# kepengxu/PGTFormer

Hardware: NVIDIA H100
Metric: clips_per_s (higher is better)
Workload: dtype bf16

## Files before the change

include/pgt_b200.h:

```cpp
#ifndef PGT_B200_H_
#define PGT_B200_H_

#include <stdint.h>

#ifdef __cplusplus
extern "C" {
#endif

typedef enum pgt_status {
  PGT_OK = 0,
  PGT_ERR_INVALID = -1,
  PGT_ERR_CUDA = -2,
  PGT_ERR_UNSUPPORTED = -3,
  PGT_ERR_DRIVER = -4
} pgt_status;

enum { PGT_BF16 = 0, PGT_F32 = 1 };
enum { PGT_ACT_NONE = 0, PGT_ACT_GELU = 1, PGT_ACT_SILU = 2, PGT_ACT_LRELU02 = 3, PGT_ACT_RELU = 4,
       PGT_ACT_SIGMOID = 5 };
enum { PGT_EPI_PLAIN = 0,
       PGT_EPI_SFT = 1 };
enum { PGT_OUT_NHWC = 0, PGT_OUT_NCHW = 1 };
enum { PGT_EPI_FLAG_RELU_AFTER_RESIDUAL = 1 };

// ... 21 lines not shown
int64_t pgt_launch_count(void);
void pgt_reset_launch_count(void);
void pgt_tmap_cache_stats(int64_t* hits, int64_t* misses);

enum { PGT_PROF_GEMM = 0, PGT_PROF_WINDOW_ATTN = 1, PGT_PROF_MHA = 2, PGT_PROF_ARGMAX = 3, PGT_PROF_ARGMIN = 4,
       PGT_PROF_NORM = 5, PGT_PROF_MOVE = 6, PGT_PROF_LAYERNORM = 7, PGT_PROF_CLASSES = 8 };
int pgt_profile_begin(void);
int pgt_profile_end(double* work, double* ms, int64_t* launches);
int pgt_profile_end_csv(const char* path, double* work, double* ms, int64_t* launches);

int pgt_linear_bf16(const void* A, int lda, const void* W, int ldw, int M, int N, int K,
                    const pgt_epilogue* ep, void* stream);

int pgt_conv_bf16(const void* x, int F, int Hin, int Win, int Cin, int ldx, const void* Wp, int ldw,
                  int Cout, int ksize, int stride, int pad_lo, const pgt_epilogue* ep, void* stream);

int pgt_conv_out_gn(const void* x, int F, int H, int W, int Cin, int ldx, const float* gn_ab, const void* Wp, int ldw,
                    int Cout, const float* bias, float* out, void* stream);
int pgt_conv_out_gn_act(const void* x, int F, int H, int W, int Cin, int ldx, const float* gn_ab, const void* Wp, int ldw,
                        int Cout, const float* bias, float* out, int silu, void* stream);

int pgt_conv_up2x_bf16(const void* x, int F, int Hin, int Win, int Cin, int ldx, const void* Wp4, int ldw,
                       int Cout, const pgt_epilogue* ep, void* stream);

int pgt_conv_rgb_bf16(const float* x_nchw, int F, int H, int W, int ksize, int stride, int pad, const float* mean3,
                      const float* std3, const void* Wp, int ldw, int Cout, const float* bias, int act, void* out,
                      int ldo, float* gn_stats, void* stream);

int64_t pgt_groupnorm_ws_floats(int F, int HW, int C);
int pgt_conv_tiles_per_frame(int Hin, int Win, int Cout, int ksize, int stride, int pad_lo);
// ... 84 lines not shown
```

pgtformer_b200/_lib.py:

```python
import ctypes
import os
from ctypes import POINTER, Structure, c_char_p, c_float, c_int, c_int32, c_int64, c_void_p

HERE = os.path.dirname(os.path.abspath(__file__))
LIB_PATH = os.path.join(HERE, 'lib', 'libpgt_b200.so')

BF16, F32 = 0, 1
ACT_NONE, ACT_GELU, ACT_SILU, ACT_LRELU02, ACT_RELU, ACT_SIGMOID = 0, 1, 2, 3, 4, 5
EPI_PLAIN, EPI_SFT = 0, 1
OUT_NHWC, OUT_NCHW = 0, 1


class Epilogue(Structure):
    _fields_ = [('bias', c_void_p), ('act', c_int32), ('mode', c_int32), ('residual', c_void_p),
                ('ldr', c_int32), ('res_dtype', c_int32), ('aux', c_void_p), ('ldaux', c_int32),
                ('sft_w', c_float), ('out', c_void_p), ('ldo', c_int32), ('out_dtype', c_int32),
                ('out_layout', c_int32), ('flags', c_int32), ('gn_stats', c_void_p)]


SIGNATURES = {
    'pgt_strerror': (c_char_p, [c_int]),
    'pgt_last_cuda_error': (c_char_p, []),
    'pgt_version': (c_int, []),
    'pgt_launch_count': (c_int64, []),
    'pgt_reset_launch_count': (None, []),
    'pgt_tmap_cache_stats': (None, [c_void_p, c_void_p]),
    'pgt_profile_begin': (c_int, []),
    'pgt_profile_end': (c_int, [c_void_p, c_void_p, c_void_p]),
    'pgt_profile_end_csv': (c_int, [c_char_p, c_void_p, c_void_p, c_void_p]),
    'pgt_linear_bf16': (c_int, [c_void_p, c_int, c_void_p, c_int, c_int, c_int, c_int, POINTER(Epilogue), c_void_p]),
    'pgt_conv_bf16': (c_int, [c_void_p, c_int, c_int, c_int, c_int, c_int, c_void_p, c_int, c_int, c_int, c_int,
                              c_int, POINTER(Epilogue), c_void_p]),
    'pgt_conv_out_gn': (c_int, [c_void_p, c_int, c_int, c_int, c_int, c_int, c_void_p, c_void_p, c_int, c_int, c_void_p,
                                c_void_p, c_void_p]),
    'pgt_conv_out_gn_act': (c_int, [c_void_p, c_int, c_int, c_int, c_int, c_int, c_void_p, c_void_p, c_int, c_int,
                                    c_void_p, c_void_p, c_int, c_void_p]),
    'pgt_groupnorm_ab': (c_int, [c_void_p, c_int, c_int, c_int, c_int, c_void_p, c_void_p, c_float, c_void_p, c_int,
                                 c_void_p, c_void_p, c_void_p]),
    'pgt_conv_up2x_bf16': (c_int, [c_void_p, c_int, c_int, c_int, c_int, c_int, c_void_p, c_int, c_int,
                                   POINTER(Epilogue), c_void_p]),
    'pgt_conv_rgb_bf16': (c_int, [c_void_p, c_int, c_int, c_int, c_int, c_int, c_int, c_void_p, c_void_p, c_void_p, c_int,
                                  c_int, c_void_p, c_int, c_void_p, c_int, c_void_p, c_void_p]),
    'pgt_groupnorm_ws_floats': (c_int64, [c_int, c_int, c_int]),
    'pgt_conv_tiles_per_frame': (c_int, [c_int, c_int, c_int, c_int, c_int, c_int]),
    'pgt_conv_tiles_exact': (c_int, [c_int, c_int, c_int, c_int, c_int, c_int]),
    'pgt_groupnorm_apply_stats': (c_int, [c_void_p, c_int, c_int, c_int, c_int, c_void_p, c_void_p, c_float, c_int,
                                          c_void_p, c_int, c_void_p, c_int, c_void_p, c_void_p]),
    'pgt_groupnorm_silu': (c_int, [c_void_p, c_int, c_int, c_int, c_int, c_void_p, c_void_p, c_float, c_int,
# ... 83 lines not shown
```

pgtformer_b200/csrc/api.cu:

```cuda
#include <atomic>
#include <cstdio>
#include <cstring>
#include <vector>

#include "common.cuh"
#include "tmap.cuh"

namespace pgt {
static thread_local char g_last_error[512] = "";
static std::atomic<long long> g_launches{0};

void set_cuda_error(cudaError_t e, const char* where) {
  snprintf(g_last_error, sizeof(g_last_error), "%s: %s (%s)", where, cudaGetErrorName(e), cudaGetErrorString(e));
}
void count_launch(int n) { g_launches.fetch_add(n, std::memory_order_relaxed); }
int num_sms() {
  static std::atomic<int> per_dev[64];
  int dev = 0;
  if (cudaGetDevice(&dev) != cudaSuccess || dev < 0 || dev >= 64) return 132;
  int n = per_dev[dev].load(std::memory_order_relaxed);
  if (n == 0) {
    if (cudaDeviceGetAttribute(&n, cudaDevAttrMultiProcessorCount, dev) != cudaSuccess || n <= 0) n = 132;
    per_dev[dev].store(n, std::memory_order_relaxed);
  }
// ... 55 lines not shown
  pgt::g_prof.clear();
  return PGT_OK;
}

extern "C" const char* pgt_strerror(int status) {
  switch (status) {
    case PGT_OK: return "ok";
    case PGT_ERR_INVALID: return "invalid argument (shape / alignment / null pointer)";
    case PGT_ERR_CUDA: return "CUDA runtime error (see pgt_last_cuda_error)";
    case PGT_ERR_UNSUPPORTED: return "configuration not covered by the sm_90a kernels";
    case PGT_ERR_DRIVER: return "cuTensorMapEncodeTiled unavailable or failed";
    default: return "unknown status";
  }
}
extern "C" const char* pgt_last_cuda_error(void) { return pgt::g_last_error; }
extern "C" int pgt_version(void) { return 202; }
extern "C" void pgt_tmap_cache_stats(int64_t* hits, int64_t* misses) {
  long long h = 0, m = 0;
  pgt::tmap_cache_stats(&h, &m);
  if (hits) *hits = h;
  if (misses) *misses = m;
}
extern "C" int64_t pgt_launch_count(void) { return pgt::g_launches.load(); }
extern "C" void pgt_reset_launch_count(void) { pgt::g_launches.store(0); }
```

pgtformer_b200/csrc/gemm_tc.cu:

```cuda
#include <cudaTypedefs.h>
#include <cstdio>
#include <cstdlib>

#include "common.cuh"
#include "tmap.cuh"
#include "ptx.cuh"
#include "epi_common.cuh"

namespace pgt {

constexpr int BM = 128;
constexpr int BK = 64;
constexpr int EPI_WARPS = 8;
constexpr int GEMM_THREADS = EPI_WARPS * 32 + 128;
constexpr int PRODUCER_WARP = EPI_WARPS;
constexpr int DMA_WARP = EPI_WARPS + 1;
constexpr int CONSUMER_REGS = 232;
constexpr int PRODUCER_REGS = 40;
static_assert(2 * 128 * CONSUMER_REGS + 128 * PRODUCER_REGS <= 65536, "register file");
constexpr int XCH_LD = 68;
constexpr int XCH_BYTES = BM * XCH_LD * 4;
constexpr int XCH_WG_LD = 36;
constexpr int XCH_WG_BYTES = BM * XCH_WG_LD * 4;
constexpr int EPI_BAR = 1;
// ... 24 lines not shown
  int act, epi_mode;
  float* gn_stats;
  int gn_cpg;
  int ntaps, tap_kw, tap_oy, tap_ox;
  int gn_tpf;
  int gn_fstride;
  int relu_after_res;
  const void* residual;
  int ldr, res_dtype;
  const void* aux;
  int ldaux;
  float sft_w;
  void* out;
  int ldo, out_dtype, out_layout;
  double flops;
};

template <int BN>
struct GemmCfg {
  static constexpr int B_STAGE_BYTES = BN * BK * 2;
  static constexpr int STAGE_BYTES = A_STAGE_BYTES + B_STAGE_BYTES;
  static constexpr int SLOTS = staging_slots<BN>();
  static constexpr int STAGING_BYTES = SLOTS * PANEL_BYTES;
  static constexpr int BUDGET = 232448 - 1024  - STAGING_BYTES - XCH_BYTES - 256 ;
  static constexpr int STAGES = (BUDGET / STAGE_BYTES) > 6 ? 6 : (BUDGET / STAGE_BYTES);
  static constexpr int SMEM_BYTES = STAGES * STAGE_BYTES + STAGING_BYTES + XCH_BYTES + 256 + 1024;
  static_assert(SMEM_BYTES <= 232448, "gemm smem budget");
};

__device__ __forceinline__ void tile_mn(const GemmParams& p, int tile, int& m_blk, int& n_blk) {
// ... 632 lines not shown
constexpr int HALO_A_BYTES = (HALO_TH + 2) * HALO_PITCH;
constexpr int HALO_A_STRIDE = ((HALO_A_BYTES + 1023) / 1024) * 1024;

template <int BN>
struct HaloCfg {
  static constexpr int B_BYTES = BN * 128;
  static constexpr int A_STAGES = 2;
  static constexpr int B_STAGES = (BN == 64) ? 9 : 4;
  static constexpr int SLOTS = staging_slots<BN>();
  static constexpr int STAGING_BYTES = SLOTS * PANEL_BYTES;
  static constexpr int XCH = 2 * XCH_WG_BYTES;
  static constexpr int SMEM_BYTES = A_STAGES * HALO_A_STRIDE + B_STAGES * B_BYTES + STAGING_BYTES + XCH + 512 + 1024;
  static_assert(SMEM_BYTES <= 232448, "halo conv smem budget");
};

template <int S>
__device__ __forceinline__ void ring_skip(int& s, uint32_t& ph, int n) {
  const int t = s + n;
  ph ^= (uint32_t)(t / S) & 1u;
  s = t % S;
}

template <int BN>
__global__ void __launch_bounds__(GEMM_THREADS, 1)
conv_halo_kernel(const __grid_constant__ CUtensorMap tmA, const __grid_constant__ CUtensorMap tmB,
                 const __grid_constant__ CUtensorMap tmO, const __grid_constant__ CUtensorMap tmR,
                 const __grid_constant__ CUtensorMap tmX, const GemmParams p) {
  using Cfg = HaloCfg<BN>;
  constexpr int AS = Cfg::A_STAGES, BS = Cfg::B_STAGES;
  constexpr int RELEASERS = 4;
  extern __shared__ uint8_t smem_raw[];
  uint8_t* smem = reinterpret_cast<uint8_t*>((reinterpret_cast<uintptr_t>(smem_raw) + 1023) & ~uintptr_t(1023));
  uint8_t* smem_a = smem;
  uint8_t* smem_b = smem + AS * HALO_A_STRIDE;
  uint8_t* staging = smem_b + BS * Cfg::B_BYTES;
  float* xch = reinterpret_cast<float*>(staging + Cfg::STAGING_BYTES);
  uint64_t* bars = reinterpret_cast<uint64_t*>(staging + Cfg::STAGING_BYTES + Cfg::XCH);
  uint64_t* a_full = bars;
  uint64_t* a_empty = bars + AS;
  uint64_t* b_full = bars + 2 * AS;
  uint64_t* b_empty = bars + 2 * AS + BS;
  uint64_t* res_bar = bars + 2 * AS + 2 * BS;
  uint64_t* slot_ready = res_bar + Cfg::SLOTS;

  const int warp = threadIdx.x >> 5;
  const int lane = threadIdx.x & 31;
  const int num_tiles = p.m_tiles * p.n_tiles;
  const int cin_pad = p.cin_blocks * BK;

  if (warp == PRODUCER_WARP && lane == 0) {
    tma_prefetch_desc(&tmA);
    tma_prefetch_desc(&tmB);
    if (p.fast_epi) tma_prefetch_desc(&tmO);
    if (p.has_res_map) tma_prefetch_desc(&tmR);
    if (p.fast_epi && p.epi_mode == PGT_EPI_SFT) tma_prefetch_desc(&tmX);
    for (int i = 0; i < AS; ++i) { mbar_init(&a_full[i], 1); mbar_init(&a_empty[i], RELEASERS); }
    for (int i = 0; i < BS; ++i) { mbar_init(&b_full[i], 1); mbar_init(&b_empty[i], RELEASERS); }
    for (int i = 0; i < Cfg::SLOTS; ++i) {
      mbar_init(&res_bar[i], 1);
      mbar_init(&slot_ready[i], RELEASERS * 32);
    }
    fence_barrier_init();
  }
  __syncthreads();

  if (warp >= EPI_WARPS) {
    setmaxnreg_dec<PRODUCER_REGS>();
    if (warp == PRODUCER_WARP) {
      int as = 0, bs = 0;
      uint32_t aph = 0, bph = 0;
      for (int tile = blockIdx.x; tile < num_tiles; tile += gridDim.x) {
        const int n_blk = tile % p.n_tiles;
        const int m_blk = tile / p.n_tiles;
        int n0, y0, x0;
        decode_conv_tile(p, m_blk, n0, y0, x0);
        {
          const int pt = tile + PREFETCH_TILES * (int)gridDim.x;
          if (BN == 64 && pt < num_tiles && elect_one()) {
            int pn0, py0, px0;
            decode_conv_tile(p, pt / p.n_tiles, pn0, py0, px0);
            for (int cb = 0; cb < p.cin_blocks; ++cb) tma_prefetch_4d(&tmA, cb * BK, px0 - 1, py0 - 1, pn0);
            if (p.has_res_map) {
              const int c0 = (pt % p.n_tiles) * BN;
              const int rw = p.out_dtype == PGT_BF16 ? 64 : 32;
              for (int c = 0; c < BN && c0 + c < p.N; c += rw) {
                tma_prefetch_4d(&tmR, c0 + c, px0, py0, pn0);
                if (p.epi_mode == PGT_EPI_SFT) tma_prefetch_4d(&tmX, c0 + c, px0, py0, pn0);
              }
            }
          }
          __syncwarp();
        }
        for (int cb = 0; cb < p.cin_blocks; ++cb) {
          mbar_wait(&a_empty[as], aph ^ 1);
          if (elect_one()) {
            mbar_arrive_expect_tx(&a_full[as], HALO_A_BYTES);
            tma_load_4d(smem_a + as * HALO_A_STRIDE, &tmA, &a_full[as], cb * BK, x0 - 1, y0 - 1, n0);
          }
          __syncwarp();
          if (++as == AS) { as = 0; aph ^= 1; }
          if (p.b_resident && tile != (int)blockIdx.x) continue;
          for (int t = 0; t < p.ntaps; ++t) {
            mbar_wait(&b_empty[bs], bph ^ 1);
            if (elect_one()) {
              mbar_arrive_expect_tx(&b_full[bs], Cfg::B_BYTES);
              tma_load_2d(smem_b + bs * Cfg::B_BYTES, &tmB, &b_full[bs], t * cin_pad + cb * BK, n_blk * BN);
            }
            __syncwarp();
            if (++bs == BS) { bs = 0; bph ^= 1; }
          }
        }
      }
      for (int i = 0; i < AS; ++i) {
        mbar_wait(&a_empty[as], aph ^ 1);
        if (++as == AS) { as = 0; aph ^= 1; }
      }
    } else if (warp == DMA_WARP) {
      const EpiCtx ctx{staging, xch, res_bar, slot_ready};
      epilogue_dma_loop<BN>(p, ctx, tmO, tmR, tmX, lane, num_tiles);
    }
  } else {
    setmaxnreg_inc<CONSUMER_REGS>();
    const int wg = warp >> 2;
    const EpiCtx ctx{staging, xch + wg * (XCH_WG_BYTES / 4), res_bar, slot_ready};
    const uint32_t a_base = smem_u32(smem_a);
    const uint32_t b_base = smem_u32(smem_b);
    constexpr uint64_t ROW_BLOCK = 8 * HALO_PITCH / 16;
    const ItemStream<BN> is(p, num_tiles);
    const int b_per_tile = p.b_resident ? 0 : p.ntaps * p.cin_blocks;
    int as = 0, bs = 0;
    uint32_t aph = 0, bph = 0;
    int k = 0;
    bool first = true;
    for (int tile = blockIdx.x, j = 0; tile < num_tiles; tile += gridDim.x, ++j) {
      const bool has_next = tile + (int)gridDim.x < num_tiles;
      const int items = p.fast_epi ? is.panels_in_tile(tile) : 0;
      if ((j & 1) != wg) {
// ... 150 lines not shown
  }
  PGT_LAUNCH_OK();
  return PGT_OK;
}

template <int BN>
static int launch_halo(const CUtensorMap& tmA, const void* W, int ldw, GemmParams& p, cudaStream_t stream) {
  using Cfg = HaloCfg<BN>;
  CUtensorMap tmB, tmO, tmR, tmX;
  int rc = encode_weight_map(&tmB, W, ldw, p.K, p.N, BN);
  if (rc != PGT_OK) return rc;
  rc = setup_epilogue_maps(p, tmA, tmO, tmR, tmX);
  if (rc != PGT_OK) return rc;
  p.n_tiles = ceil_div(p.N, BN);
  p.b_resident = (p.ntaps * p.cin_blocks <= Cfg::B_STAGES && p.n_tiles == 1) ? 1 : 0;
  static PerDeviceOnce once;
  PGT_CUDA_OK(once.run([] { return cudaFuncSetAttribute(conv_halo_kernel<BN>, cudaFuncAttributeMaxDynamicSharedMemorySize, Cfg::SMEM_BYTES); }));
  const int tiles = p.m_tiles * p.n_tiles;
  const int grid = tiles < num_sms() ? tiles : num_sms();
  {
    char desc[96];
    if (prof_enabled())
      snprintf(desc, sizeof(desc), "halo3 F%d H%d W%d K%d N%d BN%d e%d r%d", p.F, p.H, p.W, p.K, p.N, BN, p.fast_epi,
               p.b_resident);
    ProfScope ps(PGT_PROF_GEMM, p.flops, stream, desc);
    conv_halo_kernel<BN><<<grid, GEMM_THREADS, Cfg::SMEM_BYTES, stream>>>(tmA, tmB, tmO, tmR, tmX, p);
  }
  PGT_LAUNCH_OK();
  return PGT_OK;
}

static bool wide_tiles(const GemmParams& p) {
  if (p.N <= 128 || p.num_kb < 8 || p.epi_mode == PGT_EPI_SFT) return false;
  if (ceil_div(p.N, 256) * 256 > ceil_div(p.N, 128) * 128) return false;
  return p.m_tiles * ceil_div(p.N, 256) >= num_sms();
}

static int dispatch_gemm(const CUtensorMap& tmA, const void* W, int ldw, GemmParams& p, cudaStream_t stream) {
  if (p.N <= 64) return launch_gemm<64>(tmA, W, ldw, p, stream);
  if (wide_tiles(p)) return launch_gemm<256>(tmA, W, ldw, p, stream);
  return launch_gemm<128>(tmA, W, ldw, p, stream);
// ... 37 lines not shown
  p.M = M; p.N = N; p.K = K;
  p.num_kb = ceil_div(K, BK);
  p.m_tiles = ceil_div(M, BM);
  p.flops = 2.0 * M * (double)N * K;
  int rc = fill_epilogue(p, ep);
  if (rc != PGT_OK) return rc;
  CUtensorMap tmA;
  uint64_t dims[2] = {(uint64_t)K, (uint64_t)M};
  uint64_t str[1] = {(uint64_t)lda * 2};
  uint32_t box[2] = {BK, BM};
  rc = encode_map(&tmA, A, 2, dims, str, box);
  if (rc != PGT_OK) return rc;
  return dispatch_gemm(tmA, W, ldw, p, static_cast<cudaStream_t>(stream));
}

static int conv_impl(const void* x, int F, int Hin, int Win, int Cin, int ldx, const void* Wp, int ldw, int Cout,
                     int ksize, int stride, int pad_y, int pad_x, int up_phase, const pgt_epilogue* ep, void* stream) {
  const int pad_lo = pad_y;
  PGT_CHECK_ARG(x && Wp && F > 0 && Hin > 0 && Win > 0 && Cin > 0 && Cout > 0);
  PGT_CHECK_ARG((ksize >= 1 && ksize <= 3) && (stride == 1 || stride == 2) && pad_y >= 0 && pad_y <= 1 && pad_x >= 0 && pad_x <= 1);
  PGT_CHECK_ARG(stride == 1 || (ksize != 2 && pad_x == pad_y));
  PGT_CHECK_ARG((ldx % 8) == 0 && (ldw % 8) == 0 && aligned16(x) && aligned16(Wp) && ldx >= Cin);
  const int cin_pad = ceil_div(Cin, BK) * BK;
  PGT_CHECK_ARG(ldw >= ksize * ksize * cin_pad);
  GemmParams p{};
  p.N = Cout;
  p.ksize = ksize;
  p.pad_lo = pad_lo;
  p.pad_x = pad_x; p.pad_y = pad_y;
  p.cin_blocks = cin_pad / BK;
  p.K = ksize * ksize * cin_pad;
  p.num_kb = ksize * ksize * p.cin_blocks;
// ... 8 lines not shown
    p.mode = MODE_CONV_S2;
    p.H = Hin / 2; p.W = Win / 2;
    p.cin_ld = ldx;
  }
  rc = fill_epilogue(p, ep);
  if (rc != PGT_OK) return rc;
  if (up_phase >= 0) {
    if (stride != 1 || p.out_layout != PGT_OUT_NHWC || p.epi_mode != PGT_EPI_PLAIN || p.residual != nullptr)
      return PGT_ERR_UNSUPPORTED;
    const int py = up_phase >> 1, px = up_phase & 1;
    const int esz = p.out_dtype == PGT_BF16 ? 2 : 4;
    const long long Wo = 2LL * Win;
    p.out = static_cast<char*>(p.out) + ((long long)py * Wo + px) * p.ldo * esz;
    p.o_sx = 2LL * p.ldo; p.o_sy = 2LL * Wo * p.ldo; p.o_sf = 4LL * Hin * Win * p.ldo;
  }
  static const bool no_halo = getenv("PGT_NO_HALO") != nullptr;
  const bool halo = !no_halo && stride == 1 && Cout <= 128 && Hin >= HALO_TH && Win >= HALO_TW &&
                    ((up_phase < 0 && ksize == 3 && pad_y == 1 && pad_x == 1) || (up_phase >= 0 && ksize == 2));
  p.ntaps = ksize * ksize; p.tap_kw = ksize;
  p.tap_oy = up_phase >= 0 ? (up_phase >> 1) : 0;
  p.tap_ox = up_phase >= 0 ? (up_phase & 1) : 0;
  int tw = 1, th = 1, tn;
  if (halo) {
    tw = HALO_TW; th = HALO_TH;
  } else {
    while (tw * 2 <= p.W && tw * 2 <= BM) tw *= 2;
    while (th * 2 <= p.H && tw * th * 2 <= BM) th *= 2;
  }
  tn = BM / (tw * th);
  p.tw = tw; p.th = th; p.tn = tn;
  p.tiles_x = ceil_div(p.W, tw);
  p.tiles_y = ceil_div(p.H, th);
  p.m_tiles = p.tiles_x * p.tiles_y * ceil_div(F, tn);
// ... 51 lines not shown
}

extern "C" int pgt_conv_tiles_exact(int Hin, int Win, int Cout, int ksize, int stride, int pad_lo) {
  int tw, th;
  if (!conv_tile_shape(Hin, Win, Cout, ksize, stride, pad_lo, tw, th)) return 0;
  const int H = Hin / stride, W = Win / stride;
  return (W % tw == 0 && H % th == 0) ? (W / tw) * (H / th) : 0;
}

extern "C" int pgt_conv_bf16(const void* x, int F, int Hin, int Win, int Cin, int ldx, const void* Wp, int ldw,
                             int Cout, int ksize, int stride, int pad_lo, const pgt_epilogue* ep, void* stream) {
  PGT_CHECK_ARG(ksize == 1 || ksize == 3);
  return conv_impl(x, F, Hin, Win, Cin, ldx, Wp, ldw, Cout, ksize, stride, pad_lo, pad_lo, -1, ep, stream);
}

extern "C" int pgt_conv_up2x_bf16(const void* x, int F, int Hin, int Win, int Cin, int ldx, const void* Wp4, int ldw,
                                  int Cout, const pgt_epilogue* ep, void* stream) {
  PGT_CHECK_ARG(Wp4 != nullptr && ldw > 0);
  const int cin_pad = ceil_div(Cin, BK) * BK;
  PGT_CHECK_ARG(ldw >= 4 * cin_pad);
  for (int ph = 0; ph < 4; ++ph) {
    const int py = ph >> 1, px = ph & 1;
    const void* w = static_cast<const char*>(Wp4) + (size_t)ph * Cout * ldw * 2;
    int rc = conv_impl(x, F, Hin, Win, Cin, ldx, w, ldw, Cout, 2, 1, 1 - py, 1 - px, ph, ep, stream);
    if (rc != PGT_OK) return rc;
  }
  return PGT_OK;
}
```

pgtformer_b200/csrc_torch/pgt_torch_ops.cpp:

```cpp
#include <ATen/ATen.h>
#include <ATen/cuda/CUDAContext.h>
#include <c10/cuda/CUDAGuard.h>
#include <torch/library.h>

#include "../../include/pgt_b200.h"

namespace {

void check(int rc, const char* what) {
  if (rc == PGT_OK) return;
  std::string msg = std::string("libpgt_b200 (") + what + "): " + pgt_strerror(rc);
  if (rc == PGT_ERR_CUDA) msg += std::string(": ") + pgt_last_cuda_error();
  TORCH_CHECK(false, msg);
}

void* stream_of(const at::Tensor& t) { return at::cuda::getCurrentCUDAStream(t.device().index()).stream(); }

int ld(const at::Tensor& t) {
  TORCH_CHECK(t.stride(-1) == 1, "expected a channels-last tensor");
  return t.dim() > 1 ? (int)t.stride(-2) : (int)t.size(-1);
}

void window_attention(const at::Tensor& qkv, int64_t clips, int64_t H, int64_t W, int64_t C, int64_t heads, int64_t shift,
                      const at::Tensor& tab16, at::Tensor out) {
// ... 141 lines not shown
                     const c10::optional<at::Tensor>& bias, bool silu, at::Tensor out) {
  TORCH_CHECK(x.is_cuda() && x.dim() == 4 && x.scalar_type() == at::kBFloat16 && x.stride(3) == 1 &&
              x.stride(1) == x.size(2) * x.stride(2) && (x.size(0) == 1 || x.stride(0) == x.size(1) * x.stride(1)) &&
              ab.scalar_type() == at::kFloat && wp.scalar_type() == at::kBFloat16 && wp.stride(1) == 1 &&
              out.scalar_type() == at::kFloat && out.is_contiguous() && out.dim() == 4 && out.size(0) == x.size(0) &&
              out.size(1) == cout && out.size(2) == x.size(1) && out.size(3) == x.size(2),
              "conv_out_gn_act: bf16 x [F, H, W, 64], fp32 ab [F, 2, 64], bf16 packed wp, fp32 out [F, cout, H, W]");
  TORCH_CHECK(ab.device() == x.device() && wp.device() == x.device() && out.device() == x.device() &&
              (!bias.has_value() || (bias->device() == x.device() && bias->scalar_type() == at::kFloat)),
              "conv_out_gn_act: every tensor on x's device, fp32 bias");
  c10::cuda::CUDAGuard guard(x.device());
  check(pgt_conv_out_gn_act(x.data_ptr(), (int)x.size(0), (int)x.size(1), (int)x.size(2), (int)x.size(3), (int)x.stride(2),
                            ab.data_ptr<float>(), wp.data_ptr(), (int)wp.stride(0), (int)cout,
                            bias.has_value() ? bias->data_ptr<float>() : nullptr, out.data_ptr<float>(), silu ? 1 : 0,
                            stream_of(x)), "conv_out_gn_act");
}

void vq_stats(const at::Tensor& z, const at::Tensor& codebook, const at::Tensor& idx, int64_t HW, double beta,
              at::Tensor scalars, const c10::optional<at::Tensor>& zq_nchw, const c10::optional<at::Tensor>& zq_bf16,
              const c10::optional<at::Tensor>& min_enc, const c10::optional<at::Tensor>& scores,
              const c10::optional<at::Tensor>& usage) {
  TORCH_CHECK(z.is_cuda() && z.dim() == 2 && z.scalar_type() == at::kFloat && z.is_contiguous() &&
              codebook.scalar_type() == at::kFloat && codebook.is_contiguous() && codebook.dim() == 2 &&
              codebook.size(1) == z.size(1) && idx.scalar_type() == at::kLong && idx.is_contiguous() &&
              idx.numel() == z.size(0) && scalars.scalar_type() == at::kFloat && scalars.is_contiguous() &&
              scalars.numel() >= 3, "vq_stats: fp32 z [T, E], codebook [K, E], int64 idx [T], fp32 scalars [3]");
  const int64_t T = z.size(0), E = z.size(1), K = codebook.size(0);
  TORCH_CHECK(codebook.device() == z.device() && idx.device() == z.device() && scalars.device() == z.device(),
              "vq_stats: codebook, idx and scalars must be on z's device");
  auto opt = [&z](const c10::optional<at::Tensor>& t, at::ScalarType dt, int64_t n) -> void* {
// ... 20 lines not shown

TORCH_LIBRARY(pgt, m) {
  m.def("window_attention(Tensor qkv, int clips, int H, int W, int C, int heads, int shift, Tensor tab16, Tensor(a!) out) -> ()");
  m.def("mha_fwd(Tensor q, Tensor k, Tensor v, int clips, int L, int heads, int d, Tensor(a!) out) -> ()");
  m.def("argmax_gather(Tensor logits, Tensor codebook, Tensor(a!) idx, Tensor(b!) quant) -> ()");
  m.def("codebook_pack(Tensor codebook, int K) -> (Tensor, Tensor)");
  m.def("l2_argmin(Tensor z, Tensor codebook, Tensor cb16, Tensor norm, int K, Tensor(a!) idx, Tensor(b!)? quant) -> ()");
  m.def("l2_argmin_split(Tensor z, Tensor codebook, Tensor cb16, Tensor norm, int K, int splits, Tensor(a!) idx, "
        "Tensor(b!)? quant) -> ()");
  m.def("linear(Tensor a, Tensor w, Tensor? bias, int act, Tensor? residual, Tensor(a!) out) -> ()");
  m.def("soft_codes(Tensor z, Tensor codebook, Tensor norm, int K, float temp, Tensor(a!) out) -> ()");
  m.def("sample_codes(Tensor p, Tensor seed, Tensor(a!) idx) -> ()");
  m.def("rq_residual(Tensor? r_in, Tensor(a!)? r_out, Tensor idx, Tensor codebook, Tensor(b!)? agg, bool first) -> ()");
  m.def("rq_embed(Tensor idx, int d0, int d1, Tensor codebooks, Tensor(a!) out, int ldi, int ldd) -> ()");
  m.def("conv_out_gn_act(Tensor x, Tensor ab, Tensor wp, int cout, Tensor? bias, bool silu, Tensor(a!) out) -> ()");
  m.def("vq_stats(Tensor z, Tensor codebook, Tensor idx, int HW, float beta, Tensor(a!) scalars, Tensor(b!)? zq_nchw, "
        "Tensor(c!)? zq_bf16, Tensor(d!)? min_enc, Tensor(e!)? scores, Tensor(f!)? usage) -> ()");
}

TORCH_LIBRARY_IMPL(pgt, CUDA, m) {
  m.impl("window_attention", window_attention);
  m.impl("mha_fwd", mha_fwd);
  m.impl("argmax_gather", argmax_gather);
  m.impl("codebook_pack", codebook_pack);
  m.impl("l2_argmin", l2_argmin);
  m.impl("l2_argmin_split", l2_argmin_split);
  m.impl("linear", linear);
  m.impl("soft_codes", soft_codes);
  m.impl("sample_codes", sample_codes);
  m.impl("rq_residual", rq_residual);
  m.impl("rq_embed", rq_embed);
  m.impl("conv_out_gn_act", conv_out_gn_act);
  m.impl("vq_stats", vq_stats);
}
```

pgtformer_b200/engine.py:

```python
import torch
import torch.nn.functional as F

from . import ops
from .spec import Arch
from .swin3d import pack_blocks

BF = torch.bfloat16


def _on_device(fn):
    import functools

    @functools.wraps(fn)
    def wrapper(self, *a, **k):
        with torch.cuda.device(self.dev):
            return fn(self, *a, **k)
    return wrapper


def _pack_conv(w):
    co, ci, kh, kw = w.shape
    cp = (ci + 63) // 64 * 64
    wp = torch.zeros(co, kh * kw, cp, dtype=torch.float32, device=w.device)
    wp[:, :, :ci] = w.permute(0, 2, 3, 1).reshape(co, kh * kw, ci)
# ... 132 lines not shown
    def _gn_stats(self, out, chunks_per_frame):
        if chunks_per_frame <= 0 or not ops.gn_stats_supported(out.shape[-1]) or not out.is_contiguous():
            return None
        stats = self._new(out.shape[0] * chunks_per_frame * 64, dtype=torch.float32)
        out._pgt_gn = (stats, chunks_per_frame)
        return stats

    def _gn(self, x, p, silu=True):
        gn = getattr(x, '_pgt_gn', None)
        if gn is not None:
            return ops.groupnorm_apply_stats(x, self.w[p + '.weight'], self.w[p + '.bias'], self._new(*x.shape), gn[0], gn[1],
                                             silu=silu)
        return ops.groupnorm_silu(x, self.w[p + '.weight'], self.w[p + '.bias'], self._new(*x.shape), silu=silu)

    def _conv3(self, x, p, cout, out=None, gn_out=False, gn=None, gn_silu=True, **kw):
        Fr, H, W, _ = x.shape
        stride = kw.get('stride', 1)
        if gn is not None:
            x = self._gn(x, gn, silu=gn_silu)
        if out is None:
            out = self._new(Fr, H // stride, W // stride, cout)
        stats = None
        if gn_out:
            stats = self._gn_stats(out, 4 * self._stats_tiles(H, W, cout, kw.get('ksize', 3), stride, kw.get('pad_lo', 1)))
        return ops.conv(x, self.w[p + '.weight'], cout, out, bias=self.w.get(p + '.bias'), gn_stats=stats, **kw)

    def _lin(self, x, p, n, out=None, out_dtype=BF, gn_out=False, **kw):
        if out is None:
            out = self._new(*x.shape[:-1], n, dtype=out_dtype)
        stats = None
        if gn_out and out.dim() == 4 and out.dtype == BF and (out.shape[1] * out.shape[2]) % 128 == 0:
            stats = self._gn_stats(out, out.shape[1] * out.shape[2] // 32)
        return ops.linear(x, self.w[p + '.weight'], out, bias=self.w.get(p + '.bias'), N=n, gn_stats=stats, **kw)

    def td_resblock(self, x, p, cout, gn_next=False, out=None, shortcut='nin_shortcut'):
        h = self._conv3(x, p + '.conv1', cout, gn=p + '.norm1', gn_out=True)
        sc = self._lin(x, p + '.' + shortcut, cout) if (p + '.' + shortcut + '.weight') in self.w else x
        return self._conv3(h, p + '.conv2', cout, gn=p + '.norm2', residual=sc, gn_out=gn_next, out=out)

# ... 516 lines not shown
```

pgtformer_b200/ops.py:

```python
import ctypes

import torch

from . import _lib as L
from ._lib import (ACT_GELU, ACT_LRELU02, ACT_NONE, ACT_RELU, ACT_SIGMOID, ACT_SILU, BF16, EPI_PLAIN,
                   EPI_SFT, F32, OUT_NCHW, OUT_NHWC, Epilogue)


def _p(t):
    return ctypes.c_void_p(t.data_ptr()) if t is not None else None


def _stream(t=None):
    if t is not None:
        return ctypes.c_void_p(torch.cuda.current_stream(t.device).cuda_stream)
    return ctypes.c_void_p(torch.cuda.current_stream().cuda_stream)


def _dt(t):
    if t.dtype == torch.bfloat16:
        return BF16
    if t.dtype == torch.float32:
        return F32
    raise TypeError('unsupported dtype %s' % t.dtype)
# ... 58 lines not shown
    return out


def conv(x, wp, cout, out, ksize=3, stride=1, pad_lo=1, bias=None, act=ACT_NONE, residual=None, sft_scale=None,
         sft_w=0.0, nchw=False, relu_after_res=False, gn_stats=None):
    lib = L.load()
    F, H, W, Cin = x.shape
    assert x.dtype == torch.bfloat16 and x.stride(3) == 1 and x.stride(1) == W * x.stride(2) and \
        (F == 1 or x.stride(0) == H * x.stride(1))
    ep = make_epilogue(out, bias, act, residual, sft_scale, sft_w, nchw, relu_after_res, gn_stats)
    L.check(lib.pgt_conv_bf16(_p(x), F, H, W, Cin, x.stride(2), _p(wp), wp.stride(0), cout, ksize, stride, pad_lo,
                              ctypes.byref(ep), _stream()))
    return out


def conv_rgb(x_nchw, wp, bias, out, ksize, stride, pad, act=ACT_NONE, mean3=None, std3=None, gn_stats=None):
    lib = L.load()
    F, C, H, W = x_nchw.shape
    assert C == 3 and x_nchw.dtype == torch.float32 and x_nchw.is_contiguous() and wp.dtype == torch.bfloat16
    m = (ctypes.c_float * 3)(*[float(v) for v in mean3]) if mean3 is not None else None
    s = (ctypes.c_float * 3)(*[float(v) for v in std3]) if std3 is not None else None
    L.check(lib.pgt_conv_rgb_bf16(_p(x_nchw), F, H, W, ksize, stride, pad, m, s, _p(wp), wp.stride(0), wp.shape[0],
                                  _p(bias), act, _p(out), _rows(out)[2], _p(gn_stats), _stream()))
    return out


def conv_up2x(x, wp4, cout, out, bias=None, act=ACT_NONE, gn_stats=None):
    lib = L.load()
    F, H, W, Cin = x.shape
    assert x.dtype == torch.bfloat16 and wp4.dtype == torch.bfloat16 and wp4.is_contiguous() and wp4.dim() == 3
# ... 438 lines not shown
```

Measured before the change: 90.60.

## Fuse GroupNorm+SiLU on the input into the halo conv via a slab-builder warpgroup

Adds a GN variant of the halo conv kernel. An extra 128-thread builder warpgroup loads raw bf16 activations, applies the per-frame GroupNorm affine (a,b) and SiLU (as a tanh form), and writes the swizzled halo slab into shared memory instead of using a TMA load. The engine computes only the GN coefficients and skips materialising the normalised tensor for Cout<=64 3x3 convs. This removes a full read/write pass over the activations, but the extra threads raise register pressure and the SiLU math moves onto the conv's A-operand critical path.

```diff
diff --git a/include/pgt_b200.h b/include/pgt_b200.h
--- a/include/pgt_b200.h
+++ b/include/pgt_b200.h
@@ -59,6 +59,11 @@
 
 int pgt_conv_bf16(const void* x, int F, int Hin, int Win, int Cin, int ldx, const void* Wp, int ldw,
                   int Cout, int ksize, int stride, int pad_lo, const pgt_epilogue* ep, void* stream);
+
+int pgt_conv_gn_supported(int Hin, int Win, int Cin, int Cout, int ksize, int stride, int pad_lo);
+int pgt_conv_gn_bf16(const void* x, int F, int Hin, int Win, int Cin, int ldx, const void* Wp, int ldw, int Cout,
+                     int ksize, int stride, int pad_lo, const float* in_ab, int in_silu, const pgt_epilogue* ep,
+                     void* stream);
 
 int pgt_conv_out_gn(const void* x, int F, int H, int W, int Cin, int ldx, const float* gn_ab, const void* Wp, int ldw,
                     int Cout, const float* bias, float* out, void* stream);
diff --git a/pgtformer_b200/_lib.py b/pgtformer_b200/_lib.py
--- a/pgtformer_b200/_lib.py
+++ b/pgtformer_b200/_lib.py
@@ -31,7 +31,10 @@
     'pgt_linear_bf16': (c_int, [c_void_p, c_int, c_void_p, c_int, c_int, c_int, c_int, POINTER(Epilogue), c_void_p]),
     'pgt_conv_bf16': (c_int, [c_void_p, c_int, c_int, c_int, c_int, c_int, c_void_p, c_int, c_int, c_int, c_int,
                               c_int, POINTER(Epilogue), c_void_p]),
-    'pgt_conv_out_gn': (c_int, [c_void_p, c_int, c_int, c_int, c_int, c_int, c_void_p, c_void_p, c_int, c_int, c_void_p,
+    'pgt_conv_gn_supported': (c_int, [c_int, c_int, c_int, c_int, c_int, c_int, c_int]),
+    'pgt_conv_gn_bf16': (c_int, [c_void_p, c_int, c_int, c_int, c_int, c_int, c_void_p, c_int, c_int, c_int, c_int,
+                                 c_int, c_void_p, c_int, POINTER(Epilogue), c_void_p]),
+    'pgt_conv_out_gn':(c_int, [c_void_p, c_int, c_int, c_int, c_int, c_int, c_void_p, c_void_p, c_int, c_int, c_void_p,
                                 c_void_p, c_void_p]),
     'pgt_conv_out_gn_act': (c_int, [c_void_p, c_int, c_int, c_int, c_int, c_int, c_void_p, c_void_p, c_int, c_int,
                                     c_void_p, c_void_p, c_int, c_void_p]),
diff --git a/pgtformer_b200/csrc/api.cu b/pgtformer_b200/csrc/api.cu
--- a/pgtformer_b200/csrc/api.cu
+++ b/pgtformer_b200/csrc/api.cu
@@ -93,7 +93,7 @@
   }
 }
 extern "C" const char* pgt_last_cuda_error(void) { return pgt::g_last_error; }
-extern "C" int pgt_version(void) { return 202; }
+extern "C" int pgt_version(void) { return 203; }
 extern "C" void pgt_tmap_cache_stats(int64_t* hits, int64_t* misses) {
   long long h = 0, m = 0;
   pgt::tmap_cache_stats(&h, &m);
diff --git a/pgtformer_b200/csrc/gemm_tc.cu b/pgtformer_b200/csrc/gemm_tc.cu
--- a/pgtformer_b200/csrc/gemm_tc.cu
+++ b/pgtformer_b200/csrc/gemm_tc.cu
@@ -62,6 +62,9 @@
   void* out;
   int ldo, out_dtype, out_layout;
   double flops;
+  const __nv_bfloat16* gn_x;
+  const float* gn_ab;
+  int gn_ldx, gn_cin, gn_silu;
 };
 
 template <int BN>
@@ -724,6 +727,142 @@
   static_assert(SMEM_BYTES <= 232448, "halo conv smem budget");
 };
 
+constexpr int HALO_GN_THREADS = GEMM_THREADS + 128;
+constexpr int HALO_GN_BUILDER_WARP = EPI_WARPS + 4;
+constexpr int HALO_GN_CONSUMER_REGS = 168;
+static_assert(2 * 128 * HALO_GN_CONSUMER_REGS + 128 * PRODUCER_REGS + 128 * (65536 / HALO_GN_THREADS) <= 65536,
+              "register file");
+constexpr int HALO_SLAB_PIX = (HALO_TH + 2) * (HALO_TW + 2);
+constexpr int GN_SLOTS = 12;
+
+__device__ __forceinline__ int opaque(int v) {
+  asm volatile("" : "+r"(v));
+  return v;
+}
+
+template <int L, int PART>
+__device__ __forceinline__ void gn_slab_load(const GemmParams& p, int n0, int y0, int x0, int cb, int bt, uint4 (&r)[L],
+                                             uint32_t& mask) {
+  const int ch = cb * BK + (bt & 7) * 8;
+  const int prow = opaque(bt >> 3);
+  mask = 0;
+#pragma unroll
+  for (int j = 0; j < L; ++j) {
+    const int pix = prow + 16 * (PART * L + j);
+    const int sy = pix / (HALO_TW + 2), sx = pix - sy * (HALO_TW + 2);
+    const int y = y0 - 1 + sy, x = x0 - 1 + sx;
+    r[j] = make_uint4(0, 0, 0, 0);
+    if (ch < p.gn_cin && pix < HALO_SLAB_PIX && (unsigned)y < (unsigned)p.H && (unsigned)x < (unsigned)p.W) {
+      r[j] = __ldg(reinterpret_cast<const uint4*>(p.gn_x + ((size_t)(n0 * p.H + y) * p.W + x) * p.gn_ldx + ch));
+      mask |= 1u << j;
+    }
+  }
+}
+
+template <int L>
+__device__ __forceinline__ void gn_slab_convert(const GemmParams& p, uint4 (&r)[L], uint32_t mask, const float (&a)[8],
+                                                const float (&b)[8]) {
+#pragma unroll
+  for (int j = 0; j < L; ++j) {
+    uint4 o = make_uint4(0, 0, 0, 0);
+    if (mask & (1u << j)) {
+      const uint32_t u[4] = {r[j].x, r[j].y, r[j].z, r[j].w};
+      uint32_t q[4];
+#pragma unroll
+      for (int e = 0; e < 4; ++e) {
+        const float2 xv = unpack_bf16x2(u[e]);
+        float h0 = fmaf(xv.x, a[2 * e], b[2 * e]), h1 = fmaf(xv.y, a[2 * e + 1], b[2 * e + 1]);
+        if (p.gn_silu) {
+          float t0, t1;
+          asm("tanh.approx.f32 %0, %1;" : "=f"(t0) : "f"(h0));
+          asm("tanh.approx.f32 %0, %1;" : "=f"(t1) : "f"(h1));
+          h0 = fmaf(h0, t0, h0);
+          h1 = fmaf(h1, t1, h1);
+        }
+        q[e] = pack_bf16x2(h0, h1);
+      }
+      o = make_uint4(q[0], q[1], q[2], q[3]);
+    }
+    r[j] = o;
+  }
+}
+
+template <int L>
+__device__ __forceinline__ void gn_slab_store(uint32_t slab, int bt, const uint4 (&r)[L]) {
+  const int chunk = bt & 7;
+  const int prow = opaque(bt >> 3);
+#pragma unroll
+  for (int j = 0; j < L; ++j) {
+    const int pix = prow + 16 * j;
+    if (pix < HALO_SLAB_PIX) sts128(slab + pix * 128 + ((chunk ^ (pix & 7)) << 4), r[j]);
+  }
+}
+
+template <int BN>
+__device__ __forceinline__ void halo_l2_prefetch(const GemmParams& p, const CUtensorMap& tmA, const CUtensorMap& tmR,
+                                                 const CUtensorMap& tmX, int tile, int num_tiles) {
+  const int pt = tile + PREFETCH_TILES * (int)gridDim.x;
+  if (BN == 64 && pt < num_tiles && elect_one()) {
+    int pn0, py0, px0;
+    decode_conv_tile(p, pt / p.n_tiles, pn0, py0, px0);
+    for (int cb = 0; cb < p.cin_blocks; ++cb) tma_prefetch_4d(&tmA, cb * BK, px0 - 1, py0 - 1, pn0);
+    if (p.has_res_map) {
+      const int c0 = (pt % p.n_tiles) * BN;
+      const int rw = p.out_dtype == PGT_BF16 ? 64 : 32;
+      for (int c = 0; c < BN && c0 + c < p.N; c += rw) {
+        tma_prefetch_4d(&tmR, c0 + c, px0, py0, pn0);
+        if (p.epi_mode == PGT_EPI_SFT) tma_prefetch_4d(&tmX, c0 + c, px0, py0, pn0);
+      }
+    }
+  }
+  __syncwarp();
+}
+
+template <int BN>
+__device__ __forceinline__ void gn_slab_builder(const GemmParams& p, const CUtensorMap& tmA, const CUtensorMap& tmR,
+                                                const CUtensorMap& tmX, uint8_t* smem_a, uint64_t* a_full,
+                                                uint64_t* a_empty, int num_tiles) {
+  const int bt = threadIdx.x - HALO_GN_BUILDER_WARP * 32;
+  const int ch = (bt & 7) * 8;
+  int as = 0;
+  uint32_t aph = 0;
+  for (int tile = blockIdx.x; tile < num_tiles; tile += gridDim.x) {
+    if (bt < 32) halo_l2_prefetch<BN>(p, tmA, tmR, tmX, tile, num_tiles);
+    int n0, y0, x0;
+    decode_conv_tile(p, tile / p.n_tiles, n0, y0, x0);
+    for (int cb = 0; cb < p.cin_blocks; ++cb) {
+      uint4 r[GN_SLOTS];
+      uint32_t mask;
+      gn_slab_load<GN_SLOTS, 0>(p, n0, y0, x0, cb, bt, r, mask);
+      float a[8], b[8];
+      if (cb * BK + ch < p.gn_cin) {
+        const float4* pa = reinterpret_cast<const float4*>(p.gn_ab + (size_t)n0 * 2 * p.gn_cin + cb * BK + ch);
+        const float4* pb = reinterpret_cast<const float4*>(p.gn_ab + ((size_t)n0 * 2 + 1) * p.gn_cin + cb * BK + ch);
+        const float4 a0 = __ldg(pa), a1 = __ldg(pa + 1), b0 = __ldg(pb), b1 = __ldg(pb + 1);
+        a[0] = a0.x; a[1] = a0.y; a[2] = a0.z; a[3] = a0.w; a[4] = a1.x; a[5] = a1.y; a[6] = a1.z; a[7] = a1.w;
+        b[0] = b0.x; b[1] = b0.y; b[2] = b0.z; b[3] = b0.w; b[4] = b1.x; b[5] = b1.y; b[6] = b1.z; b[7] = b1.w;
+      } else {
+#pragma unroll
+        for (int j = 0; j < 8; ++j) { a[j] = 0.f; b[j] = 0.f; }
+      }
+      if (p.gn_silu) {
+#pragma unroll
+        for (int j = 0; j < 8; ++j) { a[j] *= 0.5f; b[j] *= 0.5f; }
+      }
+      gn_slab_convert<GN_SLOTS>(p, r, mask, a, b);
+      mbar_wait(&a_empty[as], aph ^ 1);
+      gn_slab_store<GN_SLOTS>(smem_u32(smem_a + as * HALO_A_STRIDE), bt, r);
+      fence_proxy_async();
+      mbar_arrive(&a_full[as]);
+      if (++as == HaloCfg<BN>::A_STAGES) { as = 0; aph ^= 1; }
+    }
+  }
+  for (int i = 0; i < HaloCfg<BN>::A_STAGES; ++i) {
+    mbar_wait(&a_empty[as], aph ^ 1);
+    if (++as == HaloCfg<BN>::A_STAGES) { as = 0; aph ^= 1; }
+  }
+}
+
 template <int S>
 __device__ __forceinline__ void ring_skip(int& s, uint32_t& ph, int n) {
   const int t = s + n;
@@ -731,12 +870,14 @@
   s = t % S;
 }
 
-template <int BN>
-__global__ void __launch_bounds__(GEMM_THREADS, 1)
+template <int BN, bool GN>
+__global__ void __launch_bounds__(GN ? HALO_GN_THREADS : GEMM_THREADS, 1)
 conv_halo_kernel(const __grid_constant__ CUtensorMap tmA, const __grid_constant__ CUtensorMap tmB,
                  const __grid_constant__ CUtensorMap tmO, const __grid_constant__ CUtensorMap tmR,
                  const __grid_constant__ CUtensorMap tmX, const GemmParams p) {
   using Cfg = HaloCfg<BN>;
+  static_assert(!GN || BN == 64, "the normalising variant exists at BN = 64");
+  constexpr int CONSUMER = GN ? HALO_GN_CONSUMER_REGS : CONSUMER_REGS;
   constexpr int AS = Cfg::A_STAGES, BS = Cfg::B_STAGES;
   constexpr int RELEASERS = 4;
   extern __shared__ uint8_t smem_raw[];
@@ -764,7 +905,7 @@
     if (p.fast_epi) tma_prefetch_desc(&tmO);
     if (p.has_res_map) tma_prefetch_desc(&tmR);
     if (p.fast_epi && p.epi_mode == PGT_EPI_SFT) tma_prefetch_desc(&tmX);
-    for (int i = 0; i < AS; ++i) { mbar_init(&a_full[i], 1); mbar_init(&a_empty[i], RELEASERS); }
+    for (int i = 0; i < AS; ++i) { mbar_init(&a_full[i], GN ? 128 : 1); mbar_init(&a_empty[i], RELEASERS); }
     for (int i = 0; i < BS; ++i) { mbar_init(&b_full[i], 1); mbar_init(&b_empty[i], RELEASERS); }
     for (int i = 0; i < Cfg::SLOTS; ++i) {
       mbar_init(&res_bar[i], 1);
@@ -774,7 +915,9 @@
   }
   __syncthreads();
 
-  if (warp >= EPI_WARPS) {
+  if (GN && warp >= HALO_GN_BUILDER_WARP) {
+    if constexpr (GN) gn_slab_builder<BN>(p, tmA, tmR, tmX, smem_a, a_full, a_empty, num_tiles);
+  } else if (warp >= EPI_WARPS) {
     setmaxnreg_dec<PRODUCER_REGS>();
     if (warp == PRODUCER_WARP) {
       int as = 0, bs = 0;
@@ -786,7 +929,7 @@
         decode_conv_tile(p, m_blk, n0, y0, x0);
         {
           const int pt = tile + PREFETCH_TILES * (int)gridDim.x;
-          if (BN == 64 && pt < num_tiles && elect_one()) {
+          if (!GN && BN == 64 && pt < num_tiles && elect_one()) {
             int pn0, py0, px0;
             decode_conv_tile(p, pt / p.n_tiles, pn0, py0, px0);
             for (int cb = 0; cb < p.cin_blocks; ++cb) tma_prefetch_4d(&tmA, cb * BK, px0 - 1, py0 - 1, pn0);
@@ -802,13 +945,15 @@
           __syncwarp();
         }
         for (int cb = 0; cb < p.cin_blocks; ++cb) {
-          mbar_wait(&a_empty[as], aph ^ 1);
-          if (elect_one()) {
-            mbar_arrive_expect_tx(&a_full[as], HALO_A_BYTES);
-            tma_load_4d(smem_a + as * HALO_A_STRIDE, &tmA, &a_full[as], cb * BK, x0 - 1, y0 - 1, n0);
+          if constexpr (!GN) {
+            mbar_wait(&a_empty[as], aph ^ 1);
+            if (elect_one()) {
+              mbar_arrive_expect_tx(&a_full[as], HALO_A_BYTES);
+              tma_load_4d(smem_a + as * HALO_A_STRIDE, &tmA, &a_full[as], cb * BK, x0 - 1, y0 - 1, n0);
+            }
+            __syncwarp();
+            if (++as == AS) { as = 0; aph ^= 1; }
           }
-          __syncwarp();
-          if (++as == AS) { as = 0; aph ^= 1; }
           if (p.b_resident && tile != (int)blockIdx.x) continue;
           for (int t = 0; t < p.ntaps; ++t) {
             mbar_wait(&b_empty[bs], bph ^ 1);
@@ -821,16 +966,18 @@
           }
         }
       }
-      for (int i = 0; i < AS; ++i) {
-        mbar_wait(&a_empty[as], aph ^ 1);
-        if (++as == AS) { as = 0; aph ^= 1; }
+      if constexpr (!GN) {
+        for (int i = 0; i < AS; ++i) {
+          mbar_wait(&a_empty[as], aph ^ 1);
+          if (++as == AS) { as = 0; aph ^= 1; }
+        }
       }
     } else if (warp == DMA_WARP) {
       const EpiCtx ctx{staging, xch, res_bar, slot_ready};
       epilogue_dma_loop<BN>(p, ctx, tmO, tmR, tmX, lane, num_tiles);
     }
   } else {
-    setmaxnreg_inc<CONSUMER_REGS>();
+    setmaxnreg_inc<CONSUMER>();
     const int wg = warp >> 2;
     const EpiCtx ctx{staging, xch + wg * (XCH_WG_BYTES / 4), res_bar, slot_ready};
     const uint32_t a_base = smem_u32(smem_a);
@@ -1011,17 +1158,27 @@
   if (rc != PGT_OK) return rc;
   p.n_tiles = ceil_div(p.N, BN);
   p.b_resident = (p.ntaps * p.cin_blocks <= Cfg::B_STAGES && p.n_tiles == 1) ? 1 : 0;
-  static PerDeviceOnce once;
-  PGT_CUDA_OK(once.run([] { return cudaFuncSetAttribute(conv_halo_kernel<BN>, cudaFuncAttributeMaxDynamicSharedMemorySize, Cfg::SMEM_BYTES); }));
+  const bool gn = p.gn_ab != nullptr;
+  if (gn && BN != 64) return PGT_ERR_UNSUPPORTED;
+  static PerDeviceOnce once, once_gn;
+  if constexpr (BN == 64) {
+    if (gn)
+      PGT_CUDA_OK(once_gn.run([] { return cudaFuncSetAttribute(conv_halo_kernel<BN, true>, cudaFuncAttributeMaxDynamicSharedMemorySize, Cfg::SMEM_BYTES); }));
+  }
+  if (!gn)
+    PGT_CUDA_OK(once.run([] { return cudaFuncSetAttribute(conv_halo_kernel<BN, false>, cudaFuncAttributeMaxDynamicSharedMemorySize, Cfg::SMEM_BYTES); }));
   const int tiles = p.m_tiles * p.n_tiles;
   const int grid = tiles < num_sms() ? tiles : num_sms();
   {
     char desc[96];
     if (prof_enabled())
-      snprintf(desc, sizeof(desc), "halo3 F%d H%d W%d K%d N%d BN%d e%d r%d", p.F, p.H, p.W, p.K, p.N, BN, p.fast_epi,
-               p.b_resident);
+      snprintf(desc, sizeof(desc), "halo3%s F%d H%d W%d K%d N%d BN%d e%d r%d", gn ? (p.gn_silu ? "_gn_silu" : "_gn") : "",
+               p.F, p.H, p.W, p.K, p.N, BN, p.fast_epi, p.b_resident);
     ProfScope ps(PGT_PROF_GEMM, p.flops, stream, desc);
-    conv_halo_kernel<BN><<<grid, GEMM_THREADS, Cfg::SMEM_BYTES, stream>>>(tmA, tmB, tmO, tmR, tmX, p);
+    if constexpr (BN == 64) {
+      if (gn) conv_halo_kernel<BN, true><<<grid, HALO_GN_THREADS, Cfg::SMEM_BYTES, stream>>>(tmA, tmB, tmO, tmR, tmX, p);
+    }
+    if (!gn) conv_halo_kernel<BN, false><<<grid, GEMM_THREADS, Cfg::SMEM_BYTES, stream>>>(tmA, tmB, tmO, tmR, tmX, p);
   }
   PGT_LAUNCH_OK();
   return PGT_OK;
@@ -1089,8 +1246,15 @@
   return dispatch_gemm(tmA, W, ldw, p, static_cast<cudaStream_t>(stream));
 }
 
+static bool takes_halo(int Hin, int Win, int Cout, int ksize, int stride, int pad_y, int pad_x, int up_phase) {
+  static const bool no_halo = getenv("PGT_NO_HALO") != nullptr;
+  return !no_halo && stride == 1 && Cout <= 128 && Hin >= HALO_TH && Win >= HALO_TW &&
+         ((up_phase < 0 && ksize == 3 && pad_y == 1 && pad_x == 1) || (up_phase >= 0 && ksize == 2));
+}
+
 static int conv_impl(const void* x, int F, int Hin, int Win, int Cin, int ldx, const void* Wp, int ldw, int Cout,
-                     int ksize, int stride, int pad_y, int pad_x, int up_phase, const pgt_epilogue* ep, void* stream) {
+                     int ksize, int stride, int pad_y, int pad_x, int up_phase, const pgt_epilogue* ep, void* stream,
+                     const float* in_ab = nullptr, int in_silu = 0) {
   const int pad_lo = pad_y;
   PGT_CHECK_ARG(x && Wp && F > 0 && Hin > 0 && Win > 0 && Cin > 0 && Cout > 0);
   PGT_CHECK_ARG((ksize >= 1 && ksize <= 3) && (stride == 1 || stride == 2) && pad_y >= 0 && pad_y <= 1 && pad_x >= 0 && pad_x <= 1);
@@ -1129,9 +1293,13 @@
     p.out = static_cast<char*>(p.out) + ((long long)py * Wo + px) * p.ldo * esz;
     p.o_sx = 2LL * p.ldo; p.o_sy = 2LL * Wo * p.ldo; p.o_sf = 4LL * Hin * Win * p.ldo;
   }
-  static const bool no_halo = getenv("PGT_NO_HALO") != nullptr;
-  const bool halo = !no_halo && stride == 1 && Cout <= 128 && Hin >= HALO_TH && Win >= HALO_TW &&
-                    ((up_phase < 0 && ksize == 3 && pad_y == 1 && pad_x == 1) || (up_phase >= 0 && ksize == 2));
+  const bool halo = takes_halo(Hin, Win, Cout, ksize, stride, pad_y, pad_x, up_phase);
+  if (in_ab != nullptr) {
+    if (!halo || up_phase >= 0 || (Cin % 8) != 0) return PGT_ERR_UNSUPPORTED;
+    p.gn_x = static_cast<const __nv_bfloat16*>(x);
+    p.gn_ab = in_ab;
+    p.gn_ldx = ldx; p.gn_cin = Cin; p.gn_silu = in_silu;
+  }
   p.ntaps = ksize * ksize; p.tap_kw = ksize;
   p.tap_oy = up_phase >= 0 ? (up_phase >> 1) : 0;
   p.tap_ox = up_phase >= 0 ? (up_phase & 1) : 0;
@@ -1213,6 +1381,19 @@
   return conv_impl(x, F, Hin, Win, Cin, ldx, Wp, ldw, Cout, ksize, stride, pad_lo, pad_lo, -1, ep, stream);
 }
 
+extern "C" int pgt_conv_gn_supported(int Hin, int Win, int Cin, int Cout, int ksize, int stride, int pad_lo) {
+  return (Cin > 0 && Cin % 8 == 0 && Cout <= 64 && takes_halo(Hin, Win, Cout, ksize, stride, pad_lo, pad_lo, -1)) ? 1 : 0;
+}
+
+extern "C" int pgt_conv_gn_bf16(const void* x, int F, int Hin, int Win, int Cin, int ldx, const void* Wp, int ldw,
+                                int Cout, int ksize, int stride, int pad_lo, const float* in_ab, int in_silu,
+                                const pgt_epilogue* ep, void* stream) {
+  PGT_CHECK_ARG(ksize == 1 || ksize == 3);
+  PGT_CHECK_ARG(in_ab != nullptr && aligned16(in_ab) && (in_silu == 0 || in_silu == 1));
+  if (!pgt_conv_gn_supported(Hin, Win, Cin, Cout, ksize, stride, pad_lo)) return PGT_ERR_UNSUPPORTED;
+  return conv_impl(x, F, Hin, Win, Cin, ldx, Wp, ldw, Cout, ksize, stride, pad_lo, pad_lo, -1, ep, stream, in_ab, in_silu);
+}
+
 extern "C" int pgt_conv_up2x_bf16(const void* x, int F, int Hin, int Win, int Cin, int ldx, const void* Wp4, int ldw,
                                   int Cout, const pgt_epilogue* ep, void* stream) {
   PGT_CHECK_ARG(Wp4 != nullptr && ldw > 0);
diff --git a/pgtformer_b200/csrc_torch/pgt_torch_ops.cpp b/pgtformer_b200/csrc_torch/pgt_torch_ops.cpp
--- a/pgtformer_b200/csrc_torch/pgt_torch_ops.cpp
+++ b/pgtformer_b200/csrc_torch/pgt_torch_ops.cpp
@@ -179,6 +179,42 @@
                             ab.data_ptr<float>(), wp.data_ptr(), (int)wp.stride(0), (int)cout,
                             bias.has_value() ? bias->data_ptr<float>() : nullptr, out.data_ptr<float>(), silu ? 1 : 0,
                             stream_of(x)), "conv_out_gn_act");
+}
+
+bool conv_gn(const at::Tensor& x, const at::Tensor& ab, bool silu, const at::Tensor& wp, int64_t cout,
+             const c10::optional<at::Tensor>& bias, const c10::optional<at::Tensor>& residual, at::Tensor out) {
+  TORCH_CHECK(x.is_cuda() && x.dim() == 4 && x.scalar_type() == at::kBFloat16 && x.stride(3) == 1 &&
+              x.stride(1) == x.size(2) * x.stride(2) && (x.size(0) == 1 || x.stride(0) == x.size(1) * x.stride(1)) &&
+              ab.scalar_type() == at::kFloat && ab.is_contiguous() && ab.numel() >= x.size(0) * 2 * x.size(3) &&
+              wp.scalar_type() == at::kBFloat16 && wp.stride(1) == 1 && out.scalar_type() == at::kBFloat16 &&
+              out.dim() == 4 && out.size(0) == x.size(0) && out.size(1) == x.size(1) && out.size(2) == x.size(2) &&
+              out.size(3) == cout,
+              "conv_gn: bf16 x [F, H, W, Cin], fp32 ab [F, 2, Cin], bf16 packed wp, bf16 out [F, H, W, cout]");
+  TORCH_CHECK(ab.device() == x.device() && wp.device() == x.device() && out.device() == x.device() &&
+              (!bias.has_value() || (bias->device() == x.device() && bias->scalar_type() == at::kFloat)) &&
+              (!residual.has_value() || (residual->device() == x.device() && residual->scalar_type() == at::kBFloat16)),
+              "conv_gn: every tensor on x's device, fp32 bias, bf16 residual");
+  c10::cuda::CUDAGuard guard(x.device());
+  pgt_epilogue ep;
+  memset(&ep, 0, sizeof(ep));
+  ep.bias = bias.has_value() ? bias->data_ptr<float>() : nullptr;
+  ep.act = PGT_ACT_NONE;
+  ep.mode = PGT_EPI_PLAIN;
+  if (residual.has_value()) {
+    ep.residual = residual->data_ptr();
+    ep.ldr = ld(*residual);
+    ep.res_dtype = PGT_BF16;
+  }
+  ep.out = out.data_ptr();
+  ep.ldo = ld(out);
+  ep.out_dtype = PGT_BF16;
+  ep.out_layout = PGT_OUT_NHWC;
+  const int rc = pgt_conv_gn_bf16(x.data_ptr(), (int)x.size(0), (int)x.size(1), (int)x.size(2), (int)x.size(3),
+                                  (int)x.stride(2), wp.data_ptr(), (int)wp.stride(0), (int)cout, 3, 1, 1,
+                                  ab.data_ptr<float>(), silu ? 1 : 0, &ep, stream_of(x));
+  if (rc == PGT_ERR_UNSUPPORTED) return false;
+  check(rc, "conv_gn");
+  return true;
 }
 
 void vq_stats(const at::Tensor& z, const at::Tensor& codebook, const at::Tensor& idx, int64_t HW, double beta,
@@ -229,6 +265,7 @@
   m.def("rq_residual(Tensor? r_in, Tensor(a!)? r_out, Tensor idx, Tensor codebook, Tensor(b!)? agg, bool first) -> ()");
   m.def("rq_embed(Tensor idx, int d0, int d1, Tensor codebooks, Tensor(a!) out, int ldi, int ldd) -> ()");
   m.def("conv_out_gn_act(Tensor x, Tensor ab, Tensor wp, int cout, Tensor? bias, bool silu, Tensor(a!) out) -> ()");
+  m.def("conv_gn(Tensor x, Tensor ab, bool silu, Tensor wp, int cout, Tensor? bias, Tensor? residual, Tensor(a!) out) -> bool");
   m.def("vq_stats(Tensor z, Tensor codebook, Tensor idx, int HW, float beta, Tensor(a!) scalars, Tensor(b!)? zq_nchw, "
         "Tensor(c!)? zq_bf16, Tensor(d!)? min_enc, Tensor(e!)? scores, Tensor(f!)? usage) -> ()");
 }
@@ -246,5 +283,6 @@
   m.impl("rq_residual", rq_residual);
   m.impl("rq_embed", rq_embed);
   m.impl("conv_out_gn_act", conv_out_gn_act);
+  m.impl("conv_gn", conv_gn);
   m.impl("vq_stats", vq_stats);
 }
diff --git a/pgtformer_b200/engine.py b/pgtformer_b200/engine.py
--- a/pgtformer_b200/engine.py
+++ b/pgtformer_b200/engine.py
@@ -170,15 +170,27 @@
         return ops.groupnorm_silu(x, self.w[p + '.weight'], self.w[p + '.bias'], self._new(*x.shape), silu=silu)
 
     def _conv3(self, x, p, cout, out=None, gn_out=False, gn=None, gn_silu=True, **kw):
-        Fr, H, W, _ = x.shape
-        stride = kw.get('stride', 1)
+        Fr, H, W, cin = x.shape
+        stride, ksize, pad_lo = kw.get('stride', 1), kw.get('ksize', 3), kw.get('pad_lo', 1)
+        ab = None
         if gn is not None:
-            x = self._gn(x, gn, silu=gn_silu)
+            if ops.conv_gn_supported(H, W, cin, cout, ksize, stride, pad_lo):
+                st = getattr(x, '_pgt_gn', None)
+                ab = ops.groupnorm_ab(x, self.w[gn + '.weight'], self.w[gn + '.bias'],
+                                      self._new(Fr * 2 * cin, dtype=torch.float32),
+                                      stats=st[0] if st else None, chunks_per_frame=st[1] if st else 0)
+            else:
+                x = self._gn(x, gn, silu=gn_silu)
         if out is None:
             out = self._new(Fr, H // stride, W // stride, cout)
         stats = None
         if gn_out:
-            stats = self._gn_stats(out, 4 * self._stats_tiles(H, W, cout, kw.get('ksize', 3), stride, kw.get('pad_lo', 1)))
+            stats = self._gn_stats(out, 4 * self._stats_tiles(H, W, cout, ksize, stride, pad_lo))
+        if ab is not None:
+            if ops.conv_gn(x, ab, self.w[p + '.weight'], cout, out, silu=gn_silu, bias=self.w.get(p + '.bias'),
+                           gn_stats=stats, **kw) is not None:
+                return out
+            x = self._gn(x, gn, silu=gn_silu)
         return ops.conv(x, self.w[p + '.weight'], cout, out, bias=self.w.get(p + '.bias'), gn_stats=stats, **kw)
 
     def _lin(self, x, p, n, out=None, out_dtype=BF, gn_out=False, **kw):
diff --git a/pgtformer_b200/ops.py b/pgtformer_b200/ops.py
--- a/pgtformer_b200/ops.py
+++ b/pgtformer_b200/ops.py
@@ -96,6 +96,26 @@
     return out
 
 
+def conv_gn_supported(H, W, cin, cout, ksize=3, stride=1, pad_lo=1):
+    return bool(L.load().pgt_conv_gn_supported(H, W, cin, cout, ksize, stride, pad_lo))
+
+
+def conv_gn(x, ab, wp, cout, out, silu=True, ksize=3, stride=1, pad_lo=1, bias=None, act=ACT_NONE, residual=None,
+            sft_scale=None, sft_w=0.0, nchw=False, relu_after_res=False, gn_stats=None):
+    lib = L.load()
+    F, H, W, Cin = x.shape
+    assert x.dtype == torch.bfloat16 and x.stride(3) == 1 and x.stride(1) == W * x.stride(2) and \
+        (F == 1 or x.stride(0) == H * x.stride(1))
+    assert ab.dtype == torch.float32 and ab.is_contiguous() and ab.numel() >= F * 2 * Cin
+    ep = make_epilogue(out, bias, act, residual, sft_scale, sft_w, nchw, relu_after_res, gn_stats)
+    rc = lib.pgt_conv_gn_bf16(_p(x), F, H, W, Cin, x.stride(2), _p(wp), wp.stride(0), cout, ksize, stride, pad_lo,
+                              _p(ab), int(silu), ctypes.byref(ep), _stream())
+    if rc == -3:
+        return None
+    L.check(rc)
+    return out
+
+
 def conv_rgb(x_nchw, wp, bias, out, ksize, stride, pad, act=ACT_NONE, mean3=None, std3=None, gn_stats=None):
     lib = L.load()
     F, C, H, W = x_nchw.shape
```

After: 92.17, median of 6. +1.7%, better.
